# Balajimcr/MuLUT

Measured on AMD Instinct MI355X. Metric: Mpixels/sec SR-x4 2-stage sdy LUT inference (HR output pixels; LR-in = value/16), higher is better.
Workload: dtype u8

## Files before the change

### mulut_amd/_native.py

```python
import ctypes
import os
import shutil
import subprocess

_PKG = os.path.dirname(os.path.abspath(__file__))
_CSRC = os.path.join(_PKG, "csrc")
_LIBDIR = os.path.join(_PKG, "lib")
LIB_PATH = os.path.join(_LIBDIR, "libmulut_hip.so")
SOURCES = ["mulut_kernels.hip", "mulut_k1.hip", "mulut_detail.hip", "mulut_capi.hip", "mulut_ft.hip", "mulut_eval.hip"]
HEADERS = ["mulut_core.h", "mulut_kernels.h", "mulut_dev.h", "mulut_tube2_asm.inc", os.path.join("..", "..", "include", "mulut.h")]
HIPCC_FLAGS = ["--offload-arch=gfx950", "-O3", "-std=c++17", "-fPIC", "-shared", "-Wall", "-Wno-inline-asm", "-Wno-pass-failed"]

EXPORTS = [
    "mulut_version", "mulut_strerror", "mulut_last_hip_error", "mulut_create", "mulut_destroy",
    "mulut_configure", "mulut_set_lut", "mulut_pass", "mulut_stage", "mulut_pipeline",
    "mulut_pipeline_rows", "mulut_halo", "mulut_reserve", "mulut_set_stage_timing", "mulut_last_stage_ms", "mulut_last_kernel_ms",
    "mulut_set_tuning", "mulut_kernel_name", "mulut_ft_stage_forward", "mulut_ft_stage_backward", "mulut_ft_quantize", "mulut_ft_quantize_backward",
    "mulut_ft_stage_forward_mask", "mulut_ft_stage_backward_mask", "mulut_eval_ws_doubles", "mulut_eval_y", "mulut_last_detail_counters", "mulut_debug_read",
]

_libs = {}


def _hipcc():
    return shutil.which("hipcc") or ("/opt/rocm/bin/hipcc" if os.path.exists("/opt/rocm/bin/hipcc") else None)


def source_hash():
    import hashlib
    h = hashlib.sha256()
    for f in sorted(SOURCES + [x for x in HEADERS if not x.endswith("mulut.h")]):
        with open(os.path.join(_CSRC, f), "rb") as fh:
            h.update(fh.read())
    return h.hexdigest()[:16]


def needs_build():
    if not os.path.exists(LIB_PATH):
        return True
    t = os.path.getmtime(LIB_PATH)
    return any(os.path.getmtime(os.path.join(_CSRC, f)) > t for f in SOURCES + HEADERS)


def audit_tube2_isa(asm_path=None):
    import re
    import tempfile
    hipcc = _hipcc()
    if hipcc is None:
        raise RuntimeError("hipcc not found: cannot audit stage_tube2_kernel")
    inc = open(os.path.join(_CSRC, "mulut_tube2_asm.inc")).read()
    row0 = int(re.search(r"#define TUBE2_ROW0 (\d+)", inc).group(1))
    with tempfile.TemporaryDirectory() as td:
        if asm_path is None:
            asm_path = os.path.join(td, "mulut_kernels.s")
            flags = [f for f in HIPCC_FLAGS if f not in ("-fPIC", "-shared")]
            subprocess.check_call([hipcc] + flags + ["--cuda-device-only", "-S", "-o", asm_path, os.path.join(_CSRC, "mulut_kernels.hip")],
                                  stderr=subprocess.DEVNULL)
        lines = open(asm_path).read().splitlines()
    reg = re.compile(r"\bv(\d+)\b|\bv\[(\d+):(\d+)\]")
    kernels, name, in_asm, bad = [], None, False, []
    for line in lines:
        m = re.match(r"^(_ZN5mulut18stage_tube2_kernel\w+):", line)
        if m:
            name, in_asm = m.group(1), False
            kernels.append(name)
            continue
        m = re.match(r"^\s*\.set (_ZN5mulut18stage_tube2_kernel\w+)\.(num_vgpr|num_agpr), (\d+)", line)
        if m:
            if (m.group(2) == "num_agpr" and int(m.group(3)) != 0) or (m.group(2) == "num_vgpr" and int(m.group(3)) > 128):
                bad.append((m.group(1), line.strip()))
            continue
        if name is None:
            continue
        if "s_endpgm" in line:
            name = None
        elif "#ASMSTART" in line:
            in_asm = True
        elif "#ASMEND" in line:
            in_asm = False
        elif not in_asm and not line.lstrip().startswith((";", ".")):
            for a, lo, hi in reg.findall(line.split(";")[0]):
                if (int(a) if a else int(hi)) >= row0:
                    bad.append((name, line.strip()))
    if len(kernels) != 3:
        raise RuntimeError("tube2 audit: expected 3 stage_tube2_kernel instances, found %d" % len(kernels))
    if bad:
        raise RuntimeError("tube2 audit failed (the compiler touched the kernel's private registers, or the register budget changed): %r" % (bad[:5],))
    return len(kernels)


def build(force=False, verbose=False):
    if not force and not needs_build():
        return LIB_PATH
    hipcc = _hipcc()
    if hipcc is None:
        raise RuntimeError("hipcc not found: cannot build libmulut_hip.so (no CPU fallback exists)")
    os.makedirs(_LIBDIR, exist_ok=True)
    tmp = "%s.%d.tmp" % (LIB_PATH, os.getpid())
    cmd = [hipcc] + HIPCC_FLAGS + ["-o", tmp] + SOURCES
    if verbose:
        print(" ".join(cmd))
    try:
        subprocess.check_call(cmd, cwd=_CSRC)
        audit_tube2_isa()
        os.replace(tmp, LIB_PATH)
    finally:
        if os.path.exists(tmp):
            os.remove(tmp)
    return LIB_PATH


def load(path=None):
    path = path or os.environ.get("MULUT_LIB") or LIB_PATH
    if path in _libs:
        return _libs[path]
    if path == LIB_PATH and needs_build():
        if os.environ.get("MULUT_NO_BUILD") == "1":
            if not os.path.exists(LIB_PATH):
                raise RuntimeError("libmulut_hip.so is missing and MULUT_NO_BUILD=1 forbids building it here")
        elif _hipcc() is not None:
            build()
        elif not os.path.exists(LIB_PATH):
            raise RuntimeError("libmulut_hip.so is missing and hipcc is unavailable; "
                               "run `python -c 'import __graft_entry__ as g; g.build()'`")
    L = ctypes.CDLL(path)
    i, p, c_char_p, i64 = ctypes.c_int, ctypes.c_void_p, ctypes.c_char_p, ctypes.c_int64
    L.mulut_version.restype = i
    L.mulut_strerror.argtypes = [i]
    L.mulut_strerror.restype = c_char_p
    L.mulut_last_hip_error.argtypes = [p]
    L.mulut_last_hip_error.restype = c_char_p
    L.mulut_create.argtypes = [i, ctypes.POINTER(p)]
    L.mulut_destroy.argtypes = [p]
    L.mulut_configure.argtypes = [p, i, c_char_p, i, i]
    L.mulut_set_lut.argtypes = [p, i, ctypes.c_char, p, i64, i]
    L.mulut_pass.argtypes = [p, i, ctypes.c_char, i, p, i, i, i, p, p]
    L.mulut_stage.argtypes = [p, i, p, i, p, i, i, i, i, i, p]
    L.mulut_pipeline.argtypes = [p, p, p, i, i, i, i, i, p]
    L.mulut_pipeline_rows.argtypes = [p, p, i, i, p, i, i, i, i, i, i, i, p]
    L.mulut_halo.argtypes = [p]
    L.mulut_reserve.argtypes = [p, i, i, i, i]
    L.mulut_set_stage_timing.argtypes = [p, i]
    L.mulut_last_stage_ms.argtypes = [p, ctypes.POINTER(ctypes.c_float), i]
    L.mulut_last_kernel_ms.argtypes = [p, ctypes.POINTER(ctypes.c_float), i]
    L.mulut_last_detail_counters.argtypes = [p, ctypes.POINTER(ctypes.c_uint32), i, p]
    L.mulut_last_detail_counters.restype = i
    L.mulut_debug_read.argtypes = [p, ctypes.POINTER(ctypes.c_uint64), i, i, p]
    L.mulut_debug_read.restype = i
    L.mulut_set_tuning.argtypes = [p, c_char_p, i]
    L.mulut_kernel_name.argtypes = [p, i]
    L.mulut_ft_stage_forward.argtypes = [i, p, c_char_p, i, i, p, i, i, i, i, p, p]
    L.mulut_ft_stage_backward.argtypes = [i, p, c_char_p, i, i, p, p, i, i, i, i, p, p, p]
    L.mulut_ft_stage_forward_mask.argtypes = [i, p, c_char_p, i, i, p, i, i, i, i, p, p, p]
    L.mulut_ft_stage_backward_mask.argtypes = [i, p, c_char_p, i, i, p, p, p, i, i, i, i, p, p, p]
    L.mulut_kernel_name.restype = c_char_p
    L.mulut_ft_quantize.argtypes = [i, p, p, i, ctypes.c_longlong, p]
    L.mulut_ft_quantize_backward.argtypes = [i, p, p, i, ctypes.c_longlong, p]
    L.mulut_eval_ws_doubles.argtypes = [i, i]
    L.mulut_eval_ws_doubles.restype = ctypes.c_longlong
    L.mulut_eval_y.argtypes = [i, p, p, i, i, i, p, ctypes.c_longlong, ctypes.POINTER(ctypes.c_double),
                               ctypes.POINTER(ctypes.c_double), p]
    L.mulut_eval_y.restype = i
    for name in ("mulut_create", "mulut_destroy", "mulut_configure", "mulut_set_lut", "mulut_pass", "mulut_stage",
                 "mulut_pipeline", "mulut_pipeline_rows", "mulut_halo", "mulut_reserve", "mulut_set_stage_timing",
                 "mulut_last_stage_ms", "mulut_last_kernel_ms", "mulut_set_tuning", "mulut_ft_stage_forward", "mulut_ft_stage_backward",
                 "mulut_ft_quantize", "mulut_ft_quantize_backward", "mulut_ft_stage_forward_mask", "mulut_ft_stage_backward_mask"):
        getattr(L, name).restype = i
    _libs[path] = L
    return L
```

### mulut_amd/csrc/mulut_kernels.hip

```cpp
#include <hip/hip_runtime.h>
#include <string.h>

#include <mutex>
#include <set>
#include <utility>

#include "mulut_dev.h"

namespace mulut {

__global__ void __launch_bounds__(256) pass_kernel(PassArgs a) {
    const long long nsite = (long long)a.C * a.H * a.W;
    const long long s = (long long)blockIdx.x * blockDim.x + threadIdx.x;
    if (s >= nsite) return;
    const int x = (int)(s % a.W);
    const int y = (int)((s / a.W) % a.H);
    const int c = (int)(s / ((long long)a.W * a.H));
    const uint8_t *pl = a.in + (long long)c * a.H * a.W;
    int v[4];
    v[0] = pl[(long long)y * a.W + x];
#pragma unroll
    for (int k = 0; k < 3; ++k) {
        int dy, dx;
        sample_offset(a.r, a.di[k], a.dj[k], dy, dx);
// ... 554 lines not shown
            finish_channel<4, OUT>(a, acc, n, c, y, x, o);
            if constexpr (OUT == kOutPackedRGBU4) {
#pragma unroll
                for (int sy = 0; sy < 4; ++sy) {
                    uint8_t *dst = const_cast<uint8_t *>(view_addr(a.out, n, 0, y * 4 + sy, x * 4)) + c;
#pragma unroll
                    for (int sx = 0; sx < 4; ++sx) dst[3 * sx] = (uint8_t)(o[sy] >> (8 * sx));
                }
            }
        }
    }
}

__global__ void __launch_bounds__(256) stage_up_fix2_kernel(StageArgs a) {
    __shared__ int s_sum[16][16];
    const uint32_t count = *a.fix_count;
    const int grp = (int)(threadIdx.x >> 4), ln = (int)(threadIdx.x & 15);
    const int ylo = imax(a.oy0 - kHalo, 0), yhi = imin(a.oy1 + kHalo, a.H) - 1;
    const int unbias = 128 * kQ * 4 * a.M - a.bias_num;
    for (uint32_t i = blockIdx.x * 16u + (uint32_t)grp; i < count; i += gridDim.x * 16u) {
        const uint32_t ent = a.fix_list[i], id = ent & 0x3FFFFFFFu, only = ent >> 30;
        const int x = (int)(id % (uint32_t)a.W), y = (int)((id / (uint32_t)a.W) % (uint32_t)a.H), n = (int)(id / ((uint32_t)a.W * (uint32_t)a.H));
        if (n >= a.N || y < a.oy0 || y >= a.oy1) continue;
        const int c_lo = only == 3u ? 0 : (int)only, c_hi = only == 3u ? imin(a.C, 3) : imin((int)only + 1, a.C);
        for (int c = c_lo; c < c_hi; ++c) {
            s_sum[grp][ln] = 0;
            __builtin_amdgcn_fence(__ATOMIC_RELEASE, "wavefront");
            auto px = [&](int dy, int dx) {
                const int gy = imin(imax(y + dy, ylo), yhi), gx = imin(imax(x + dx, 0), a.W - 1);
                return (int)*view_addr(a.in, n, c, gy, gx);
            };
            const int va = px(0, 0);
            for (int p = ln; p < 4 * a.M; p += 16) {
                const int m = p >> 2, r = p & 3;
                int dy, dx, v[3];
#pragma unroll
                for (int k = 0; k < 3; ++k) {
                    sample_offset(r, a.di[m][k], a.dj[m][k], dy, dx);
                    v[k] = px(dy, dx);
                }
                int idx[5], w[5];
                simplex4(va, v[0], v[1], v[2], idx, w);
                const uint4 *tab = (const uint4 *)a.lut[m];
                uint32_t row[5][4];
#pragma unroll
                for (int j = 0; j < 5; ++j) {
                    const uint4 t = tab[idx[j]];
                    row[j][0] = t.x; row[j][1] = t.y; row[j][2] = t.z; row[j][3] = t.w;
                }
#pragma unroll
                for (int e = 0; e < 16; ++e) {
                    int sum = 0;
#pragma unroll
                    for (int j = 0; j < 5; ++j) sum += w[j] * (int)((row[j][e >> 2] >> (8 * (e & 3))) & 0xFFu);
                    const int pos = r == 0 ? e : r == 1 ? (e & 3) * 4 + 3 - (e >> 2) : r == 2 ? 15 - e : (3 - (e & 3)) * 4 + (e >> 2);
                    atomicAdd(&s_sum[grp][pos], sum);
                }
            }
            __builtin_amdgcn_fence(__ATOMIC_ACQ_REL, "wavefront");
            const uint32_t b = rhe_clip_u8(s_sum[grp][ln] - unbias, a.div);
            *const_cast<uint8_t *>(view_addr(a.out, n, c, y * 4 + (ln >> 2), x * 4 + (ln & 3))) = (uint8_t)b;
            __builtin_amdgcn_fence(__ATOMIC_ACQ_REL, "wavefront");
        }
    }
}

__global__ void __launch_bounds__(256) stage_up_fix3_kernel(StageArgs a) {
    __shared__ int s_sum[16][16];
    const uint32_t count = *a.fix_count;
    const int grp = (int)(threadIdx.x >> 4), ln = (int)(threadIdx.x & 15);
    const int ylo = imax(a.oy0 - kHalo, 0), yhi = imin(a.oy1 + kHalo, a.H) - 1;
    const int unbias = 128 * kQ * 4 * a.M - a.bias_num;
    const uint32_t stride = gridDim.x * 16u;
    constexpr uint32_t kNone = 0xFFFFFFFFu;
    struct Pix { int x, y, n, va, v[3]; };
    auto decode = [&](uint32_t ent, int &x, int &y, int &n) {
        const uint32_t id = ent & 0x3FFFFFFFu;
        x = (int)(id % (uint32_t)a.W); y = (int)((id / (uint32_t)a.W) % (uint32_t)a.H); n = (int)(id / ((uint32_t)a.W * (uint32_t)a.H));
    };
    auto fetch = [&](uint32_t ent, int c, Pix &p) {
        if (ent == kNone) return;
        decode(ent, p.x, p.y, p.n);
        auto px = [&](int dy, int dx) {
            const int gy = imin(imax(p.y + dy, ylo), yhi), gx = imin(imax(p.x + dx, 0), a.W - 1);
            return (int)*view_addr(a.in, p.n, c, gy, gx);
        };
        p.va = px(0, 0);
        if (ln < 4 * a.M) {
            const int m = ln >> 2, r = ln & 3;
#pragma unroll
            for (int k = 0; k < 3; ++k) {
                int dy, dx;
                sample_offset(r, a.di[m][k], a.dj[m][k], dy, dx);
                p.v[k] = px(dy, dx);
            }
        }
    };
    auto finish = [&](const Pix &p, int c) {
        s_sum[grp][ln] = 0;
        __builtin_amdgcn_fence(__ATOMIC_RELEASE, "wavefront");
        for (int q = ln; q < 4 * a.M; q += 16) {
            const int m = q >> 2, r = q & 3;
            int v[3] = {p.v[0], p.v[1], p.v[2]};
            if (q != ln) {
                auto px = [&](int dy, int dx) {
                    const int gy = imin(imax(p.y + dy, ylo), yhi), gx = imin(imax(p.x + dx, 0), a.W - 1);
                    return (int)*view_addr(a.in, p.n, c, gy, gx);
                };
#pragma unroll
                for (int k = 0; k < 3; ++k) {
                    int dy, dx;
                    sample_offset(r, a.di[m][k], a.dj[m][k], dy, dx);
                    v[k] = px(dy, dx);
                }
            }
            int idx[5], w[5];
            simplex4(p.va, v[0], v[1], v[2], idx, w);
            const uint4 *tab = (const uint4 *)a.lut[m];
            uint32_t row[5][4];
#pragma unroll
            for (int j = 0; j < 5; ++j) {
                const uint4 t = tab[idx[j]];
                row[j][0] = t.x; row[j][1] = t.y; row[j][2] = t.z; row[j][3] = t.w;
            }
#pragma unroll
            for (int e = 0; e < 16; ++e) {
                int sum = 0;
#pragma unroll
                for (int j = 0; j < 5; ++j) sum += w[j] * (int)((row[j][e >> 2] >> (8 * (e & 3))) & 0xFFu);
                const int pos = r == 0 ? e : r == 1 ? (e & 3) * 4 + 3 - (e >> 2) : r == 2 ? 15 - e : (3 - (e & 3)) * 4 + (e >> 2);
                atomicAdd(&s_sum[grp][pos], sum);
            }
        }
        __builtin_amdgcn_fence(__ATOMIC_ACQ_REL, "wavefront");
        const uint32_t b = rhe_clip_u8(s_sum[grp][ln] - unbias, a.div);
        *const_cast<uint8_t *>(view_addr(a.out, p.n, c, p.y * 4 + (ln >> 2), p.x * 4 + (ln & 3))) = (uint8_t)b;
        __builtin_amdgcn_fence(__ATOMIC_ACQ_REL, "wavefront");
    };
    auto first_channel = [&](uint32_t ent) { return (ent >> 30) == 3u ? 0 : (int)(ent >> 30); };

    uint32_t i = blockIdx.x * 16u + (uint32_t)grp;
    uint32_t ent_cur = i < count ? a.fix_list[i] : kNone;
    uint32_t ent_nxt = i + stride < count && i + stride >= i ? a.fix_list[i + stride] : kNone;
    Pix cur, nxt;
    cur.x = cur.y = cur.n = cur.va = 0; cur.v[0] = cur.v[1] = cur.v[2] = 0;
    nxt = cur;
    if (ent_cur != kNone) fetch(ent_cur, first_channel(ent_cur), cur);
    while (ent_cur != kNone) {
        const uint32_t i2 = i + 2u * stride;
        const uint32_t ent_nn = (i2 < count && i2 >= i) ? a.fix_list[i2] : kNone;
        if (ent_nxt != kNone) fetch(ent_nxt, first_channel(ent_nxt), nxt);
        const int c0 = first_channel(ent_cur);
        finish(cur, c0);
        if ((ent_cur >> 30) == 3u)
            for (int c = 1; c < a.C; ++c) {
                Pix p;
                p.v[0] = p.v[1] = p.v[2] = 0;
                fetch(ent_cur, c, p);
                finish(p, c);
            }
        ent_cur = ent_nxt; cur = nxt; ent_nxt = ent_nn; i += stride;
    }
}

hipError_t launch_stage_up_fix(const StageArgs &a, int out_mode, int num_cus, hipStream_t st, int variant) {
    if (a.C > 3 || !a.fix_list || !a.fix_count) return hipErrorInvalidValue;
    const dim3 grid((unsigned)(4 * num_cus)), block(256);
    if (a.M > 4 && variant == 1) variant = 0;
    if (variant == 0) hipLaunchKernelGGL(stage_up_fix2_kernel, dim3((unsigned)(8 * num_cus)), block, 0, st, a);
    else if (variant == 2) hipLaunchKernelGGL(stage_up_fix3_kernel, dim3((unsigned)(8 * num_cus)), block, 0, st, a);
    else if (out_mode == kOutPlanarU4) hipLaunchKernelGGL((stage_up_fix_kernel<kOutPlanarU4>), grid, block, 0, st, a);
    else if (out_mode == kOutPackedRGBU4 && a.C == 3) hipLaunchKernelGGL((stage_up_fix_kernel<kOutPackedRGBU4>), grid, block, 0, st, a);
    else hipLaunchKernelGGL((stage_up_fix_kernel<kOutGeneric>), grid, block, 0, st, a);
    return hipGetLastError();
}

const char *stage_tube_name(int out_mode) {
    return out_mode == kOutPackedRGBU4 ? "stage_tube_kernel<rgb>" : out_mode == kOutPlanarU4 ? "stage_tube_kernel<planar>"
                                                                                              : "stage_tube_kernel<generic>";
}

template <int OUT>
static hipError_t launch_tube_t(const StageArgs &a, const BandArgs &b, int num_cus, hipStream_t st) {
    auto kern = stage_tube_kernel<OUT, KB_TW, KB_TH>;
    {
        const hipError_t e = raise_lds_limit((const void *)kern, 160 * 1024);
        if (e != hipSuccess) return e;
    }
    const long long ntiles = (long long)a.N * a.tiles_x * a.tiles_y;
    if (ntiles <= 0 || ntiles > 0x7fffffffLL) return hipErrorInvalidValue;
    const unsigned grid = (unsigned)(ntiles < num_cus ? ntiles : num_cus);
    hipLaunchKernelGGL(kern, dim3(grid), dim3(KB_TW * KB_TH), (size_t)kTubeLdsBytes, st, a, b);
    return hipGetLastError();
}

hipError_t launch_stage_tube(const StageArgs &a, const BandArgs &b, int out_mode, int num_cus, hipStream_t st) {
    if (a.C > 3 || a.M > 3) return hipErrorInvalidValue;
    if (out_mode == kOutPlanarU4) return launch_tube_t<kOutPlanarU4>(a, b, num_cus, st);
    if (out_mode == kOutPackedRGBU4 && a.C == 3) return launch_tube_t<kOutPackedRGBU4>(a, b, num_cus, st);
    return launch_tube_t<kOutGeneric>(a, b, num_cus, st);
}

#if defined(MULUT_TUBE2_ASM_INC)
#include MULUT_TUBE2_ASM_INC
#else
#include "mulut_tube2_asm.inc"
#endif

struct T2Pair {
    uint32_t base, s0, s1, s2;
    uint32_t w0, w1, w2, w3, w4;
};
__host__ __device__ constexpr int t2_modes(int pats) { return pats & 3; }
__host__ __device__ constexpr int t2_pat(int pats, int m) { return (pats >> (2 + 2 * m)) & 3; }
constexpr int kT2W = 16, kT2H = 4;
constexpr int kT2PW = kT2W + 2 * kTubeHaloX, kT2PH = kT2H + 2 * kHalo, kT2Chan = 2 * kT2PH * kT2PW;
constexpr int kT2WaveTileBytes = 3 * kT2Chan;
constexpr int kT2FixCap = 3 * kT2W * kT2H;
constexpr int kT2FixOff = 3 * kTubeBandBytes + 16 * kT2WaveTileBytes + 2 * 16 * KB_TW * KB_TH;
constexpr int kTube2LdsBytes = kT2FixOff + 16 * kT2FixCap * 4 + 16;
static_assert(kTube2LdsBytes <= 160 * 1024, "LDS budget");
static_assert(KB_TW % kT2W == 0 && KB_TH % kT2H == 0 && (KB_TW / kT2W) * (KB_TH / kT2H) == 16 && KB_TW / kT2W == 4, "16 wave tiles per verdict tile, four across");
__host__ __device__ constexpr int t2_nb(int pat, int r, int k, int sign) {
    return 2 * ((2 + sign * rot_dy(r, kPatDi[pat][k], kPatDj[pat][k])) * kT2PW + 2 + sign * rot_dx(r, kPatDi[pat][k], kPatDj[pat][k]));
}
__host__ __device__ constexpr int t2_imm(int pat) { return pat * kTubeBandBytes - tube_bias(pat); }

__device__ __forceinline__ float t2_f32_of_i16(uint32_t x) {
    float f;
    asm("v_cvt_f32_i32_sdwa %0, sext(%1) dst_sel:DWORD dst_unused:UNUSED_PAD src0_sel:WORD_0" : "=v"(f) : "v"(x));
    return f;
}

template <int PAT>
__device__ __forceinline__ void t2_index(uint32_t k0, uint32_t ha, uint32_t base_a0, uint32_t pb, uint32_t pc, uint32_t pd, T2Pair &o, uint32_t &dirty) {
    constexpr uint32_t SB = kTubeSB * 16, SC = kTubeSC * 16, SD = kTubeSD * 16;
    uint32_t k1 = pb | pk_dup(SB), k2 = pc | pk_dup(SC), k3 = pd | pk_dup(SD);
    const uint32_t hb = pb & 0x000F000Fu, hc = pc & 0x000F000Fu, hd = pd & 0x000F000Fu;
    pk_cmpx_desc(k0, k1);
    pk_cmpx_desc(k2, k3);
    pk_cmpx_desc(k0, k2);
    pk_cmpx_desc(k1, k3);
    pk_cmpx_desc(k1, k2);
    const uint32_t f1 = pk_shr12(k0), f2 = pk_shr12(k1), f3 = pk_shr12(k2), f4 = pk_shr12(k3);
    o.base = pk_mad(pb, pk_dup(SB), pk_mad(pc, pk_dup(SC), pk_mad(pd, pk_dup(SD), base_a0 + pk_dup((uint32_t)tube_bias(PAT)))));
    o.s0 = k0 & 0x0FF00FF0u;
    o.s1 = k1 & 0x0FF00FF0u;
    o.s2 = k2 & 0x0FF00FF0u;
    o.w0 = pk_dup(kQ) - f1;
    o.w1 = f1 - f2;
    o.w2 = f2 - f3;
    o.w3 = f3 - f4;
    o.w4 = f4;
    const uint32_t mx = pk_max(pk_max(hb, hc), pk_max(hd, ha));
    const uint32_t mn = pk_min(pk_min(hb, hc), pk_min(hd, ha));
    dirty |= (mx - mn) & 0xFFFEFFFEu;
}

#define T2_ACC_OPS(lo, hi) [l0] "+v"(lo[0]), [l1] "+v"(lo[1]), [l2] "+v"(lo[2]), [l3] "+v"(lo[3]), [h0] "+v"(hi[0]), [h1] "+v"(hi[1]), [h2] "+v"(hi[2]), [h3] "+v"(hi[3])
#define T2_TMP_OPS [a0] "=&v"(a0), [a1] "=&v"(a1), [a2] "=&v"(a2), [a3] "=&v"(a3)
#define T2_W_OPS(c) [w0] "v"(c.w0), [w1] "v"(c.w1), [w2] "v"(c.w2), [w3] "v"(c.w3), [w4] "v"(c.w4)
#define T2_ADDR_OPS(n) [base] "v"(n.base), [s0] "v"(n.s0), [s1] "v"(n.s1), [s2] "v"(n.s2)
#define T2_IMM_OPS(PAT) [ilo] "i"(t2_imm(PAT)), [ihi] "i"(t2_imm(PAT) + kTubePlaneBytes), [ilo4] "i"(t2_imm(PAT) + kTubeAll * 16), [ihi4] "i"(t2_imm(PAT) + kTubeAll * 16 + kTubePlaneBytes)
#define T2_NB_OPS(PAT, R, OFF) [n0] "i"(t2_nb(PAT, R, 0, 1) + (OFF)), [n1] "i"(t2_nb(PAT, R, 0, -1) + (OFF)), [n2] "i"(t2_nb(PAT, R, 1, 1) + (OFF)), \
    [n3] "i"(t2_nb(PAT, R, 1, -1) + (OFF)), [n4] "i"(t2_nb(PAT, R, 2, 1) + (OFF)), [n5] "i"(t2_nb(PAT, R, 2, -1) + (OFF)), [nan] "i"(2 * (2 * kT2PW + 2) + (OFF))

#define T2_NBOUT_OPS [pb] "=&v"(pb), [pc] "=&v"(pc), [pd] "=&v"(pd), [t0] "=&v"(t0), [t1] "=&v"(t1), [t2] "=&v"(t2)
template <int PAT>
__device__ __forceinline__ void t2_block_a(uint32_t (&lo)[4], uint32_t (&hi)[4], const T2Pair &cur) {
    uint32_t a0, a1, a2, a3;
    asm volatile(TUBE2_ASM_A : T2_ACC_OPS(lo, hi), T2_TMP_OPS : T2_W_OPS(cur), T2_ADDR_OPS(cur), T2_IMM_OPS(PAT) : TUBE2_CLOBBERS);
}
template <int NPAT, int NN, int TPAT, int TR, int TOFF, bool LAST>
__device__ __forceinline__ void t2_block_b(uint32_t (&lo)[4], uint32_t (&hi)[4], const T2Pair &cur, const T2Pair &nxt, uint32_t win,
                                           uint32_t &pb, uint32_t &pc, uint32_t &pd, uint32_t &ca) {
    uint32_t a0, a1, a2, a3, t0, t1, t2;
    if constexpr (LAST)
        asm volatile(TUBE2_ASM_B_LAST : T2_ACC_OPS(lo, hi) : T2_W_OPS(cur) : TUBE2_CLOBBERS);
    else if constexpr (NN == 0)
        asm volatile(TUBE2_ASM_B_N0 : T2_ACC_OPS(lo, hi), T2_TMP_OPS : T2_W_OPS(cur), T2_ADDR_OPS(nxt), T2_IMM_OPS(NPAT) : TUBE2_CLOBBERS);
    else if constexpr (NN == 6)
        asm volatile(TUBE2_ASM_B_N6 : T2_ACC_OPS(lo, hi), T2_TMP_OPS, T2_NBOUT_OPS : T2_W_OPS(cur), T2_ADDR_OPS(nxt), T2_IMM_OPS(NPAT), [win] "v"(win), T2_NB_OPS(TPAT, TR, TOFF) : TUBE2_CLOBBERS);
    else
        asm volatile(TUBE2_ASM_B_N7 : T2_ACC_OPS(lo, hi), T2_TMP_OPS, T2_NBOUT_OPS, [ca] "=&v"(ca) : T2_W_OPS(cur), T2_ADDR_OPS(nxt), T2_IMM_OPS(NPAT), [win] "v"(win), T2_NB_OPS(TPAT, TR, TOFF) : TUBE2_CLOBBERS);
}

template <int OUT, int PATS>
__global__ void __launch_bounds__(KB_TW *KB_TH) __attribute__((amdgpu_waves_per_eu(TUBE2_WAVES_PER_EU, TUBE2_WAVES_PER_EU))) stage_tube2_kernel(StageArgs a, BandArgs b) {
    constexpr int TW = KB_TW, TH = KB_TH, PW = kT2PW, PH = kT2PH, NT = TW * TH;
    constexpr int M = t2_modes(PATS), NP = 2 * M;
    constexpr int DW = PW / 4, PER4 = (3 * PH * DW + 63) / 64;
    extern __shared__ __attribute__((aligned(16))) uint8_t smem[];
    uint32_t *s_next = (uint32_t *)(smem + kTube2LdsBytes - 16);
    if (lds_addr_of(smem) != 0u) __builtin_trap();

    const int ntiles = a.N * a.tiles_x * a.tiles_y;
    const int G = gridDim.x;
    const bool by_xcd = (G & 7) == 0;
    const int per = (ntiles + 7) >> 3;
    const int first = by_xcd ? (int)(blockIdx.x & 7) * per + (int)(blockIdx.x >> 3) : (int)blockIdx.x;
    const int last = by_xcd ? imin(((int)(blockIdx.x & 7) + 1) * per, ntiles) : ntiles;
    const int step = by_xcd ? (G >> 3) : G;
    if (first >= last) return;
    const int ylo = imax(a.oy0 - kHalo, 0), yhi = imin(a.oy1 + kHalo, a.H) - 1;
    const bool dw_ok = __builtin_amdgcn_readfirstlane((int)(a.in.sX == 1 && ((a.W | a.in.sY | a.in.sC) & 3) == 0 && (a.in.sN & 3) == 0 && (((uintptr_t)a.in.p) & 3) == 0)) != 0;
    const int wave = __builtin_amdgcn_readfirstlane((int)(threadIdx.x >> 6));
    uint8_t *img = smem + 3 * kTubeBandBytes + wave * kT2WaveTileBytes;

    auto grab = [&]() {
        for (;;) {
            uint32_t j = 0;
            if ((threadIdx.x & 63) == 0) j = atomicAdd(s_next, 1u);
            j = (uint32_t)__builtin_amdgcn_readfirstlane((int)j);
            const long long tile = (long long)first + (long long)(j >> 4) * step;
            if (tile >= last) return -1;
            if (a.verdict_take >= 0 && (int)a.verdict[tile] != a.verdict_take) continue;
            int n, ty0, tx0;
            decode_tile(a, (int)tile, n, ty0, tx0, TW, TH);
            if (tx0 + kT2W * (int)(j & 3u) >= a.W || ty0 + kT2H * (int)((j >> 2) & 3u) >= a.oy1) continue;
            return (int)j;
        }
    };
    auto origin = [&](int j, int &n, int &y0, int &x0) {
        decode_tile(a, first + (j >> 4) * step, n, y0, x0, TW, TH);
        x0 += kT2W * (j & 3);
        y0 += kT2H * ((j >> 2) & 3);
    };
    auto fetch = [&](int j, uint32_t (&v)[PER4]) {
        if (!dw_ok || j < 0) return;
        int n, y0, x0;
        origin(j, n, y0, x0);
        int lane = (int)(threadIdx.x & 63);
        asm volatile("" : "+v"(lane));
#pragma unroll
        for (int k = 0; k < PER4; ++k) {
            const int i = lane + 64 * k;
            const int q = i % DW, py = (i / DW) % PH, c = imin(i / (DW * PH), a.C - 1);
            const int gy = imin(imax(y0 + py - kHalo, ylo), yhi);
            const int gx = imin(imax(x0 - kTubeHaloX + 4 * q, 0), a.W - 4);
            v[k] = *(const uint32_t *)view_addr(a.in, n, c, gy, gx);
        }
    };
    auto stash = [&](int j, const uint32_t (&v)[PER4]) {
        if (j < 0) return;
        int n, y0, x0;
        origin(j, n, y0, x0);
        int lane = (int)(threadIdx.x & 63);
        asm volatile("" : "+v"(lane));
        if (dw_ok) {
            const bool edge = __builtin_amdgcn_readfirstlane((int)(x0 - kTubeHaloX < 0 || x0 - kTubeHaloX + 4 * (DW - 1) > a.W - 4)) != 0;
#pragma unroll
            for (int k = 0; k < PER4; ++k) {
                const int i = lane + 64 * k;
                if (i < a.C * PH * DW) {
                    uint32_t lo, hi;
                    if (!edge) {
                        lo = __builtin_amdgcn_perm(0u, v[k], 0x0C010C00u); hi = __builtin_amdgcn_perm(0u, v[k], 0x0C030C02u);
                    } else {
                        const int gx = x0 - kTubeHaloX + 4 * (i % DW);
                        const uint32_t sel_lo = gx < 0 ? 0x0C000C00u : gx > a.W - 4 ? 0x0C030C03u : 0x0C010C00u;
                        const uint32_t sel_hi = gx < 0 ? 0x0C000C00u : gx > a.W - 4 ? 0x0C030C03u : 0x0C030C02u;
                        lo = __builtin_amdgcn_perm(0u, v[k], sel_lo); hi = __builtin_amdgcn_perm(0u, v[k], sel_hi);
                    }
                    uint2 c2;
                    c2.x = pk_mad(lo, pk_dup(0x1000u), pk_shr4(lo));
                    c2.y = pk_mad(hi, pk_dup(0x1000u), pk_shr4(hi));
                    *(uint2 *)(img + 8 * i) = c2;
                }
            }
        } else {
            for (int i = lane; i < a.C * PH * PW; i += 64) {
                const int px = i % PW, py = (i / PW) % PH, c = i / (PW * PH);
                const int gy = imin(imax(y0 + py - kHalo, ylo), yhi);
                const int gx = imin(imax(x0 + px - kTubeHaloX, 0), a.W - 1);
                ((uint16_t *)img)[i] = (uint16_t)pixel_code1(*view_addr(a.in, n, c, gy, gx));
            }
        }
    };

#if defined(MULUT_VARIANT_t2prof)
    const unsigned long long t_first = __builtin_amdgcn_s_memtime(), r_first = __builtin_amdgcn_s_memrealtime();
    uint32_t t_prev = (uint32_t)t_first, t_ph0 = 0, t_ph1 = 0, t_ph2 = 0, t_ph3 = 0, t_ph4 = 0, t_ph5 = 0;
#define T2_STAMP(PH) do { const uint32_t t_now = (uint32_t)__builtin_amdgcn_s_memtime(); t_ph##PH += t_now - t_prev; t_prev = t_now; } while (0)
#elif defined(MULUT_T2_MARKERS)
#define T2_STAMP(PH) asm volatile("; MULUT_T2_PHASE_END " #PH)
#else
#define T2_STAMP(PH) do { } while (0)
#endif
    static_for<0, M>([&](auto MI) {
        constexpr int pat = t2_pat(PATS, MI);
        const uint4 *src = (const uint4 *)b.band[MI];
        uint4 *dst = (uint4 *)(smem + pat * kTubeBandBytes);
        const uint32_t k = b.scale[MI];
        if (k == 0x00010001u) {
            for (int i = threadIdx.x; i < kTubeBandBytes / 16; i += NT) dst[i] = src[i];
        } else {
            for (int i = threadIdx.x; i < kTubeBandBytes / 16; i += NT) {
                const uint4 v = src[i];
                dst[i] = make_uint4(pk_mad(v.x, k, 0u), pk_mad(v.y, k, 0u), pk_mad(v.z, k, 0u), pk_mad(v.w, k, 0u));
            }
        }
    });
    if (threadIdx.x == 0) *s_next = 0u;
    __syncthreads();
    T2_STAMP(5);

    uint32_t *fix_buf = (uint32_t *)(smem + kT2FixOff) + wave * kT2FixCap;
    uint32_t fix_have = 0u;
    auto fix_flush = [&]() {
        if (fix_have == 0u) return;
        const unsigned long long act = __ballot(true);
        const uint32_t rank = (uint32_t)__popcll(act & ((1ull << (threadIdx.x & 63)) - 1ull)), nact = (uint32_t)__popcll(act);
        uint32_t at = 0u;
        if (rank == 0u) at = atomicAdd(a.fix_count, fix_have);
        at = (uint32_t)__builtin_amdgcn_readfirstlane((int)at);
        __builtin_amdgcn_fence(__ATOMIC_ACQ_REL, "wavefront");
        for (uint32_t i = rank; i < fix_have; i += nact) a.fix_list[at + i] = fix_buf[i];
        __builtin_amdgcn_fence(__ATOMIC_ACQ_REL, "wavefront");
        fix_have = 0u;
    };
    uint32_t pix[PER4];
    int item = grab();
    fetch(item, pix);
    stash(item, pix);
    while (item >= 0) {
        const int nxt_item = grab();
        fetch(nxt_item, pix);
        auto site = [&](int &n_, int &y_, int &x_, int &lx_, int &ly_) {
            int y0, x0;
            origin(item, n_, y0, x0);
            int l = (int)(threadIdx.x & 63);
            asm volatile("" : "+v"(l));
            lx_ = l % kT2W; ly_ = l / kT2W;
            y_ = y0 + ly_; x_ = x0 + lx_;
        };
        int n, y, x, lx, ly;
        site(n, y, x, lx, ly);
        T2_STAMP(0);
        if (y < a.oy1 && x < a.W) {
            uint32_t win = (uint32_t)(3 * kTubeBandBytes + wave * kT2WaveTileBytes + 2 * (ly * PW + lx + kTubeHaloX - kHalo));
            auto park = [&]() {
                int t = (int)threadIdx.x;
                asm volatile("" : "+v"(t));
                return (uint4 *)(smem + 3 * kTubeBandBytes + 16 * kT2WaveTileBytes) + t;
            };
            uint32_t dmask = 0u, dirty = 0u, dirty_n = 0u;
            uint32_t o[4] = {0u, 0u, 0u, 0u};
            uint32_t pb, pc, pd, ca;
            uint32_t k0, ha, ba0;
            auto anchor = [&](uint32_t c2) {
                k0 = (c2 & 0xF000F000u) | pk_dup((uint32_t)kTubeSA * 16);
                ha = c2 & 0x000F000Fu;
                ba0 = pk_mad(c2, pk_dup((uint32_t)kTubeSA * 16), 0u);
            };
            T2Pair cur, nxt;
            {
                constexpr int p0 = t2_pat(PATS, 0);
                uint32_t t0, t1, t2;
                asm volatile(TUBE2_ASM_LOAD_NB_ANCHOR : T2_NBOUT_OPS, [ca] "=&v"(ca) : [win] "v"(win), T2_NB_OPS(p0, 0, 0) : TUBE2_CLOBBERS);
                anchor(ca);
                t2_index<p0>(k0, ha, ba0, pb, pc, pd, cur, dirty);
                asm volatile(TUBE2_ASM_LOAD_NB : T2_NBOUT_OPS : [win] "v"(win), T2_NB_OPS(p0, 1, 0) : TUBE2_CLOBBERS);
                uint32_t a0, a1, a2, a3;
                asm volatile(TUBE2_ASM_FIRST_ROWS : T2_TMP_OPS : T2_ADDR_OPS(cur), T2_IMM_OPS(p0) : TUBE2_CLOBBERS);
                t2_index<p0>(k0, ha, ba0, pb, pc, pd, nxt, dirty);
            }
            RotAcc<4> acc;
            const bool wide = a.M > 4;
            auto acc_start = [&]() {
                acc.clear();
                if (OUT != kOutGeneric && !wide) {
                    const uint32_t nb = pk_dup((uint32_t)(65536 - 128 * kQ * 4 * a.M));
#pragma unroll
                    for (int k = 0; k < 4; ++k) acc.lo02[k] = acc.hi02[k] = nb;
                }
            };
            acc_start();
            T2_STAMP(1);
#pragma clang loop unroll(disable)
            for (int c = 0; c < a.C; ++c, win += kT2Chan) {
                const bool more = c + 1 < a.C;
                asm volatile("; MULUT_T2_STREAM_BEGIN (tools/ubench/gen_stream_ubench.py cuts the ISA here)");
                static_for<0, NP>([&](auto PI) {
                    constexpr int p = PI;
                    if constexpr (p == (NP >= 6 ? 4 : NP - 1)) asm volatile("; MULUT_T2_STREAM_END");
                    constexpr int pat = t2_pat(PATS, p >> 1), R = p & 1;
                    constexpr bool t_here = p + 2 < NP;
                    constexpr int tp = t_here ? p + 2 : p + 2 - NP, tpat = t2_pat(PATS, tp >> 1), tr = tp & 1, toff = t_here ? 0 : kT2Chan;
                    constexpr bool n_here = p + 1 < NP;
                    constexpr int npat = t2_pat(PATS, n_here ? (p + 1) >> 1 : 0);
                    T2Pair nn;
                    auto &lo = R == 0 ? acc.lo02 : acc.lo13;
                    auto &hi = R == 0 ? acc.hi02 : acc.hi13;
                    t2_block_a<pat>(lo, hi, cur);
                    if (t_here || more) {
                        t2_block_b<npat, (tp == 0 ? 7 : 6), tpat, tr, toff, false>(lo, hi, cur, nxt, win, pb, pc, pd, ca);
                        if constexpr (tp == 0) anchor(ca);
                        if constexpr (t_here) t2_index<tpat>(k0, ha, ba0, pb, pc, pd, nn, dirty);
                        else t2_index<tpat>(k0, ha, ba0, pb, pc, pd, nn, dirty_n);
                    } else {
                        if constexpr (n_here) t2_block_b<npat, 0, 0, 0, 0, false>(lo, hi, cur, nxt, win, pb, pc, pd, ca);
                        else t2_block_b<npat, 0, 0, 0, 0, true>(lo, hi, cur, nxt, win, pb, pc, pd, ca);
                        nn = nxt;
                    }
                    cur = nxt;
                    nxt = nn;
                });
                if (wide) {
                    tube_finish_rows_wide(a, acc, o);
                    if constexpr (OUT == kOutPackedRGBU4) {
                        if (c < 2) park()[c * NT] = make_uint4(o[0], o[1], o[2], o[3]);
                    } else {
                        int n2, y2, x2, lx2, ly2;
                        site(n2, y2, x2, lx2, ly2);
#pragma unroll
                        for (int sy = 0; sy < 4; ++sy) {
                            if constexpr (OUT == kOutPlanarU4) {
                                *(uint32_t *)const_cast<uint8_t *>(view_addr(a.out, n2, c, y2 * 4 + sy, x2 * 4)) = o[sy];
                            } else {
#pragma unroll
                                for (int sx = 0; sx < 4; ++sx) *const_cast<uint8_t *>(view_addr(a.out, n2, c, y2 * 4 + sy, x2 * 4 + sx)) = (uint8_t)(o[sy] >> (8 * sx));
                            }
                        }
                    }
                } else if constexpr (OUT != kOutGeneric) {
                    static_for<0, 4>([&](auto SY) {
                        constexpr int sy = SY;
                        const uint32_t s0 = tube_field<4 * sy + 0>(acc.lo02, acc.hi02) + tube_field<12 + sy>(acc.lo13, acc.hi13);
                        const uint32_t s1 = tube_field<4 * sy + 1>(acc.lo02, acc.hi02) + tube_field<8 + sy>(acc.lo13, acc.hi13);
                        const uint32_t s2 = tube_field<4 * sy + 2>(acc.lo02, acc.hi02) + tube_field<4 + sy>(acc.lo13, acc.hi13);
                        const uint32_t s3 = tube_field<4 * sy + 3>(acc.lo02, acc.hi02) + tube_field<0 + sy>(acc.lo13, acc.hi13);
                        uint32_t r = __builtin_amdgcn_cvt_pk_u8_f32(t2_f32_of_i16(s0) * a.inv_d, 0u, 0u);
                        r = __builtin_amdgcn_cvt_pk_u8_f32(t2_f32_of_i16(s1) * a.inv_d, 1u, r);
                        r = __builtin_amdgcn_cvt_pk_u8_f32(t2_f32_of_i16(s2) * a.inv_d, 2u, r);
                        r = __builtin_amdgcn_cvt_pk_u8_f32(t2_f32_of_i16(s3) * a.inv_d, 3u, r);
                        o[sy] = r;
                    });
                    if constexpr (OUT == kOutPackedRGBU4) {
                        if (c < 2) park()[c * NT] = make_uint4(o[0], o[1], o[2], o[3]);
                    } else {
                        int n2, y2, x2, lx2, ly2;
                        site(n2, y2, x2, lx2, ly2);
#pragma unroll
                        for (int sy = 0; sy < 4; ++sy) *(uint32_t *)const_cast<uint8_t *>(view_addr(a.out, n2, c, y2 * 4 + sy, x2 * 4)) = o[sy];
                    }
                } else {
                    int n2, y2, x2, lx2, ly2;
                    site(n2, y2, x2, lx2, ly2);
                    finish_channel<4, OUT>(a, acc, n2, c, y2, x2, o);
                }
                acc_start();
                dmask |= (dirty != 0u ? 1u : 0u) << c;
                dirty = dirty_n;
                dirty_n = 0u;
            }
            T2_STAMP(2);
            site(n, y, x, lx, ly);
            if constexpr (OUT == kOutPackedRGBU4) {
                const uint4 r = park()[0], g = park()[NT];
                const uint32_t oR[4] = {r.x, r.y, r.z, r.w}, oG[4] = {g.x, g.y, g.z, g.w};
                store_rgb<4>(a, n, y, x, oR, oG, o);
            }
#if defined(MULUT_VARIANT_nofixlist)
            if (dmask == 0xFFFFFFFFu) a.fix_list[0] = 0u;
#else
            if (__ballot(dmask != 0u) != 0ull) {
                const uint32_t pixel_id = (uint32_t)((n * a.H + y) * a.W + x);
                const unsigned long long m0 = __ballot((dmask & 1u) != 0u), m1 = __ballot((dmask & 2u) != 0u), m2 = __ballot((dmask & 4u) != 0u);
                const uint32_t n0 = (uint32_t)__popcll(m0), n1 = (uint32_t)__popcll(m1), n2 = (uint32_t)__popcll(m2);
                if (fix_have + n0 + n1 + n2 > (uint32_t)kT2FixCap) fix_flush();
                const unsigned long long below = (1ull << (threadIdx.x & 63)) - 1ull;
                if (dmask & 1u) fix_buf[fix_have + (uint32_t)__popcll(m0 & below)] = pixel_id;
                if (dmask & 2u) fix_buf[fix_have + n0 + (uint32_t)__popcll(m1 & below)] = pixel_id | (1u << 30);
                if (dmask & 4u) fix_buf[fix_have + n0 + n1 + (uint32_t)__popcll(m2 & below)] = pixel_id | (2u << 30);
                fix_have += n0 + n1 + n2;
            }
#endif
        }
        T2_STAMP(3);
        stash(nxt_item, pix);
        T2_STAMP(4);
        item = nxt_item;
    }
    fix_flush();
#if defined(MULUT_VARIANT_t2prof)
    if (a.dbg && (threadIdx.x & 63) == 0) {
        atomicAdd(a.dbg + 0, (unsigned long long)t_ph0); atomicAdd(a.dbg + 1, (unsigned long long)t_ph1); atomicAdd(a.dbg + 2, (unsigned long long)t_ph2);
        atomicAdd(a.dbg + 3, (unsigned long long)t_ph3); atomicAdd(a.dbg + 4, (unsigned long long)t_ph4); atomicAdd(a.dbg + 5, (unsigned long long)t_ph5);
        atomicAdd(a.dbg + 6, __builtin_amdgcn_s_memtime() - t_first);
        atomicAdd(a.dbg + 7, __builtin_amdgcn_s_memrealtime() - r_first);
        atomicAdd(a.dbg + 8, 1ull);
    }
#endif
#undef T2_STAMP
}

constexpr int kT2PatsSDY = 3 | (0 << 2) | (1 << 4) | (2 << 6);

static bool tube2_counts(const StageArgs &a, int (&cnt)[3]) {
    cnt[0] = cnt[1] = cnt[2] = 0;
    for (int m = 0; m < a.M; ++m) {
        int di[3], dj[3], p = -1;
        for (int q = 0; q < 3 && p < 0; ++q) {
            pattern_offsets("sdy"[q], di, dj);
            if (memcmp(di, a.di[m], sizeof(di)) == 0 && memcmp(dj, a.dj[m], sizeof(dj)) == 0) p = q;
        }
        if (p < 0) return false;
        ++cnt[p];
    }
    return true;
}
bool stage_tube2_supported(const StageArgs &a) {
    int cnt[3];
    return a.C <= 3 && a.M <= kMaxTube2Modes && tube2_counts(a, cnt) && cnt[0] && cnt[1] && cnt[2] && (a.M > 4 || a.use_f32) &&
           a.bias_num == 0;
}

template <int OUT>
static hipError_t launch_tube2_t(const StageArgs &a, const BandArgs &b, int num_cus, hipStream_t st) {
    auto kern = stage_tube2_kernel<OUT, kT2PatsSDY>;
    {
        const hipError_t e = raise_lds_limit((const void *)kern, 160 * 1024);
        if (e != hipSuccess) return e;
    }
    const long long ntiles = (long long)a.N * a.tiles_x * a.tiles_y;
    if (ntiles <= 0 || ntiles > 0x7fffffffLL) return hipErrorInvalidValue;
    const unsigned grid = (unsigned)(ntiles < num_cus ? ntiles : num_cus);
    hipLaunchKernelGGL(kern, dim3(grid), dim3(KB_TW * KB_TH), (size_t)kTube2LdsBytes, st, a, b);
    return hipGetLastError();
}

hipError_t launch_stage_tube2(const StageArgs &a, const BandArgs &bm, int out_mode, int num_cus, hipStream_t st) {
    int cnt[3];
    if (!stage_tube2_supported(a) || !tube2_counts(a, cnt)) return hipErrorInvalidValue;
    BandArgs b;
    memset(&b, 0, sizeof(b));
    for (int m = 0; m < a.M; ++m) {
        const int p = a.dj[m][0] == 2 ? 1 : a.di[m][0] == 1 ? 2 : 0;
        b.band[p] = bm.band[m];
        b.scale[p] = (uint32_t)cnt[p] * 0x00010001u;
    }
    if (out_mode == kOutPlanarU4) return launch_tube2_t<kOutPlanarU4>(a, b, num_cus, st);
    if (out_mode == kOutPackedRGBU4 && a.C == 3) return launch_tube2_t<kOutPackedRGBU4>(a, b, num_cus, st);
    return launch_tube2_t<kOutGeneric>(a, b, num_cus, st);
}

}
```

Measured before the change: 144,100.

## Reload tube2 kernel args from kernarg segment to cut SGPR/VGPR pressure

Replaces values held across the tube2 loop (dw_ok, ylo/yhi, decoded tile bases) with on-demand scalar loads from the kernarg segment pointer. Fetch and stash now use one lane per (row, dword) with a per-channel inner loop, and output addresses use 32-bit offsets with inlined RGB interleaved stores. The fix-list flush assumes a full wave and the ballot is moved outside the in-bounds branch so all lanes take part. The aim is lower register pressure and cheaper address math, at the cost of more scalar loads and a new restriction that the batch strides fit in 31 bits.

```diff
diff --git a/mulut_amd/_native.py b/mulut_amd/_native.py
--- a/mulut_amd/_native.py
+++ b/mulut_amd/_native.py
@@ -72,7 +72,7 @@
             continue
         if name is None:
             continue
-        if "s_endpgm" in line:
+        if line.startswith(".Lfunc_end"):
             name = None
         elif "#ASMSTART" in line:
             in_asm = True
diff --git a/mulut_amd/csrc/mulut_kernels.hip b/mulut_amd/csrc/mulut_kernels.hip
--- a/mulut_amd/csrc/mulut_kernels.hip
+++ b/mulut_amd/csrc/mulut_kernels.hip
@@ -880,11 +880,30 @@
     const int last = by_xcd ? imin(((int)(blockIdx.x & 7) + 1) * per, ntiles) : ntiles;
     const int step = by_xcd ? (G >> 3) : G;
     if (first >= last) return;
-    const int ylo = imax(a.oy0 - kHalo, 0), yhi = imin(a.oy1 + kHalo, a.H) - 1;
-    const bool dw_ok = __builtin_amdgcn_readfirstlane((int)(a.in.sX == 1 && ((a.W | a.in.sY | a.in.sC) & 3) == 0 && (a.in.sN & 3) == 0 && (((uintptr_t)a.in.p) & 3) == 0)) != 0;
+    typedef const __attribute__((address_space(4))) StageArgs KArgs;
+    auto kargs = [&]() {
+        uint64_t p = (uint64_t)(uintptr_t)__builtin_amdgcn_kernarg_segment_ptr();
+        asm volatile("" : "+s"(p));
+        const uint32_t lo = (uint32_t)__builtin_amdgcn_readfirstlane((int)(uint32_t)p), hi = (uint32_t)__builtin_amdgcn_readfirstlane((int)(uint32_t)(p >> 32));
+        return (KArgs *)(uintptr_t)(((uint64_t)hi << 32) | lo);
+    };
+    auto dw_ok = [&]() {
+        KArgs *k = kargs();
+        return k->in.sX == 1 && ((k->W | k->in.sY | k->in.sC) & 3) == 0 && (k->in.sN & 3) == 0 && (((uintptr_t)k->in.p) & 3) == 0;
+    };
     const int wave = __builtin_amdgcn_readfirstlane((int)(threadIdx.x >> 6));
     uint8_t *img = smem + 3 * kTubeBandBytes + wave * kT2WaveTileBytes;
 
+    auto origin = [&](int j, int &n, int &y0, int &x0) {
+        KArgs *k = kargs();
+        int b = first + (j >> 4) * step;
+        const int tx = b % k->tiles_x;
+        b /= k->tiles_x;
+        const int ty = b % k->tiles_y;
+        n = b / k->tiles_y;
+        y0 = k->oy0 + ty * TH + kT2H * ((j >> 2) & 3);
+        x0 = tx * TW + kT2W * (j & 3);
+    };
     auto grab = [&]() {
         for (;;) {
             uint32_t j = 0;
@@ -892,61 +911,67 @@
             j = (uint32_t)__builtin_amdgcn_readfirstlane((int)j);
             const long long tile = (long long)first + (long long)(j >> 4) * step;
             if (tile >= last) return -1;
-            if (a.verdict_take >= 0 && (int)a.verdict[tile] != a.verdict_take) continue;
-            int n, ty0, tx0;
-            decode_tile(a, (int)tile, n, ty0, tx0, TW, TH);
-            if (tx0 + kT2W * (int)(j & 3u) >= a.W || ty0 + kT2H * (int)((j >> 2) & 3u) >= a.oy1) continue;
+            KArgs *k = kargs();
+            if (k->verdict_take >= 0 && (int)k->verdict[tile] != k->verdict_take) continue;
+            int n, y0, x0;
+            origin((int)j, n, y0, x0);
+            if (x0 >= k->W || y0 >= k->oy1) continue;
             return (int)j;
         }
     };
-    auto origin = [&](int j, int &n, int &y0, int &x0) {
-        decode_tile(a, first + (j >> 4) * step, n, y0, x0, TW, TH);
-        x0 += kT2W * (j & 3);
-        y0 += kT2H * ((j >> 2) & 3);
-    };
+    static_assert(PH * 8 == 64 && DW <= 8 && PER4 == 3, "one lane per (image row, dword) of a channel; one dword per channel and lane");
     auto fetch = [&](int j, uint32_t (&v)[PER4]) {
-        if (!dw_ok || j < 0) return;
+        if (j < 0 || !dw_ok()) return;
         int n, y0, x0;
         origin(j, n, y0, x0);
-        int lane = (int)(threadIdx.x & 63);
+        KArgs *k = kargs();
+        const int ylo = imax(k->oy0 - kHalo, 0), yhi = imin(k->oy1 + kHalo, k->H) - 1;
+        uint32_t lane = threadIdx.x & 63u;
         asm volatile("" : "+v"(lane));
-#pragma unroll
-        for (int k = 0; k < PER4; ++k) {
-            const int i = lane + 64 * k;
-            const int q = i % DW, py = (i / DW) % PH, c = imin(i / (DW * PH), a.C - 1);
-            const int gy = imin(imax(y0 + py - kHalo, ylo), yhi);
-            const int gx = imin(imax(x0 - kTubeHaloX + 4 * q, 0), a.W - 4);
-            v[k] = *(const uint32_t *)view_addr(a.in, n, c, gy, gx);
+        const uint32_t q = lane & 7u, py = lane >> 3;
+        if (q < (uint32_t)DW) {
+            const int gy = imin(imax(y0 + (int)py - kHalo, ylo), yhi);
+            const int gx = imin(imax(x0 - kTubeHaloX + 4 * (int)q, 0), k->W - 4);
+            const uint32_t off = (uint32_t)(gy - k->in.row0) * (uint32_t)k->in.sY + (uint32_t)gx;
+            const uint8_t *plane = k->in.p + (long long)n * k->in.sN;
+#pragma unroll
+            for (int c = 0; c < PER4; ++c) v[c] = *(const uint32_t *)(plane + (long long)imin(c, k->C - 1) * k->in.sC + off);
         }
     };
     auto stash = [&](int j, const uint32_t (&v)[PER4]) {
         if (j < 0) return;
         int n, y0, x0;
         origin(j, n, y0, x0);
-        int lane = (int)(threadIdx.x & 63);
-        asm volatile("" : "+v"(lane));
-        if (dw_ok) {
-            const bool edge = __builtin_amdgcn_readfirstlane((int)(x0 - kTubeHaloX < 0 || x0 - kTubeHaloX + 4 * (DW - 1) > a.W - 4)) != 0;
-#pragma unroll
-            for (int k = 0; k < PER4; ++k) {
-                const int i = lane + 64 * k;
-                if (i < a.C * PH * DW) {
-                    uint32_t lo, hi;
-                    if (!edge) {
-                        lo = __builtin_amdgcn_perm(0u, v[k], 0x0C010C00u); hi = __builtin_amdgcn_perm(0u, v[k], 0x0C030C02u);
-                    } else {
-                        const int gx = x0 - kTubeHaloX + 4 * (i % DW);
-                        const uint32_t sel_lo = gx < 0 ? 0x0C000C00u : gx > a.W - 4 ? 0x0C030C03u : 0x0C010C00u;
-                        const uint32_t sel_hi = gx < 0 ? 0x0C000C00u : gx > a.W - 4 ? 0x0C030C03u : 0x0C030C02u;
-                        lo = __builtin_amdgcn_perm(0u, v[k], sel_lo); hi = __builtin_amdgcn_perm(0u, v[k], sel_hi);
+        KArgs *k = kargs();
+        if (dw_ok()) {
+            uint32_t lane = threadIdx.x & 63u;
+            asm volatile("" : "+v"(lane));
+            const uint32_t q = lane & 7u, py = lane >> 3;
+            if (q < (uint32_t)DW) {
+                const int W = k->W;
+                const bool edge = x0 - kTubeHaloX < 0 || x0 - kTubeHaloX + 4 * (DW - 1) > W - 4;
+                uint32_t sel_lo = 0x0C010C00u, sel_hi = 0x0C030C02u;
+                if (edge) {
+                    const int gx = x0 - kTubeHaloX + 4 * (int)q;
+                    sel_lo = gx < 0 ? 0x0C000C00u : gx > W - 4 ? 0x0C030C03u : 0x0C010C00u;
+                    sel_hi = gx < 0 ? 0x0C000C00u : gx > W - 4 ? 0x0C030C03u : 0x0C030C02u;
+                }
+                uint2 *dst = (uint2 *)img + (py * DW + q);
+#pragma unroll
+                for (int c = 0; c < PER4; ++c) {
+                    if (c < k->C) {
+                        const uint32_t lo = __builtin_amdgcn_perm(0u, v[c], sel_lo), hi = __builtin_amdgcn_perm(0u, v[c], sel_hi);
+                        uint2 c2;
+                        c2.x = pk_mad(lo, pk_dup(0x1000u), pk_shr4(lo));
+                        c2.y = pk_mad(hi, pk_dup(0x1000u), pk_shr4(hi));
+                        dst[c * PH * DW] = c2;
                     }
-                    uint2 c2;
-                    c2.x = pk_mad(lo, pk_dup(0x1000u), pk_shr4(lo));
-                    c2.y = pk_mad(hi, pk_dup(0x1000u), pk_shr4(hi));
-                    *(uint2 *)(img + 8 * i) = c2;
                 }
             }
         } else {
+            int lane = (int)(threadIdx.x & 63);
+            asm volatile("" : "+v"(lane));
+            const int ylo = imax(a.oy0 - kHalo, 0), yhi = imin(a.oy1 + kHalo, a.H) - 1;
             for (int i = lane; i < a.C * PH * PW; i += 64) {
                 const int px = i % PW, py = (i / PW) % PH, c = i / (PW * PH);
                 const int gy = imin(imax(y0 + py - kHalo, ylo), yhi);
@@ -987,8 +1012,7 @@
     uint32_t fix_have = 0u;
     auto fix_flush = [&]() {
         if (fix_have == 0u) return;
-        const unsigned long long act = __ballot(true);
-        const uint32_t rank = (uint32_t)__popcll(act & ((1ull << (threadIdx.x & 63)) - 1ull)), nact = (uint32_t)__popcll(act);
+        const uint32_t rank = threadIdx.x & 63u, nact = 64u;
         uint32_t at = 0u;
         if (rank == 0u) at = atomicAdd(a.fix_count, fix_have);
         at = (uint32_t)__builtin_amdgcn_readfirstlane((int)at);
@@ -996,6 +1020,10 @@
         for (uint32_t i = rank; i < fix_have; i += nact) a.fix_list[at + i] = fix_buf[i];
         __builtin_amdgcn_fence(__ATOMIC_ACQ_REL, "wavefront");
         fix_have = 0u;
+    };
+    auto out_off = [&](int y_, int x_) {
+        KArgs *k = kargs();
+        return (uint32_t)(4 * y_ - k->out.row0) * (uint32_t)k->out.sY + (uint32_t)(4 * x_) * (uint32_t)k->out.sX;
     };
     uint32_t pix[PER4];
     int item = grab();
@@ -1015,6 +1043,7 @@
         int n, y, x, lx, ly;
         site(n, y, x, lx, ly);
         T2_STAMP(0);
+        uint32_t dmask = 0u;
         if (y < a.oy1 && x < a.W) {
             uint32_t win = (uint32_t)(3 * kTubeBandBytes + wave * kT2WaveTileBytes + 2 * (ly * PW + lx + kTubeHaloX - kHalo));
             auto park = [&]() {
@@ -1022,7 +1051,7 @@
                 asm volatile("" : "+v"(t));
                 return (uint4 *)(smem + 3 * kTubeBandBytes + 16 * kT2WaveTileBytes) + t;
             };
-            uint32_t dmask = 0u, dirty = 0u, dirty_n = 0u;
+            uint32_t dirty = 0u, dirty_n = 0u;
             uint32_t o[4] = {0u, 0u, 0u, 0u};
             uint32_t pb, pc, pd, ca;
             uint32_t k0, ha, ba0;
@@ -1120,7 +1149,7 @@
                         int n2, y2, x2, lx2, ly2;
                         site(n2, y2, x2, lx2, ly2);
 #pragma unroll
-                        for (int sy = 0; sy < 4; ++sy) *(uint32_t *)const_cast<uint8_t *>(view_addr(a.out, n2, c, y2 * 4 + sy, x2 * 4)) = o[sy];
+                        for (int sy = 0; sy < 4; ++sy) *(uint32_t *)(a.out.p + (long long)n2 * a.out.sN + (long long)c * a.out.sC + (out_off(y2, x2) + (uint32_t)sy * (uint32_t)a.out.sY)) = o[sy];
                     }
                 } else {
                     int n2, y2, x2, lx2, ly2;
@@ -1137,24 +1166,36 @@
             if constexpr (OUT == kOutPackedRGBU4) {
                 const uint4 r = park()[0], g = park()[NT];
                 const uint32_t oR[4] = {r.x, r.y, r.z, r.w}, oG[4] = {g.x, g.y, g.z, g.w};
-                store_rgb<4>(a, n, y, x, oR, oG, o);
-            }
+                KArgs *k = kargs();
+                uint8_t *plane = k->out.p + (long long)n * k->out.sN;
+                const uint32_t off = out_off(y, x), sY = (uint32_t)k->out.sY;
+#pragma unroll
+                for (int sy = 0; sy < 4; ++sy) {
+                    uint32_t w0, w1, w2;
+                    interleave_rgb4(oR[sy], oG[sy], o[sy], w0, w1, w2);
+                    uint32_t *dst = (uint32_t *)(plane + (off + (uint32_t)sy * sY));
+                    dst[0] = w0;
+                    dst[1] = w1;
+                    dst[2] = w2;
+                }
+            }
+        }
 #if defined(MULUT_VARIANT_nofixlist)
-            if (dmask == 0xFFFFFFFFu) a.fix_list[0] = 0u;
+        if (dmask == 0xFFFFFFFFu) a.fix_list[0] = 0u;
 #else
-            if (__ballot(dmask != 0u) != 0ull) {
-                const uint32_t pixel_id = (uint32_t)((n * a.H + y) * a.W + x);
-                const unsigned long long m0 = __ballot((dmask & 1u) != 0u), m1 = __ballot((dmask & 2u) != 0u), m2 = __ballot((dmask & 4u) != 0u);
-                const uint32_t n0 = (uint32_t)__popcll(m0), n1 = (uint32_t)__popcll(m1), n2 = (uint32_t)__popcll(m2);
-                if (fix_have + n0 + n1 + n2 > (uint32_t)kT2FixCap) fix_flush();
-                const unsigned long long below = (1ull << (threadIdx.x & 63)) - 1ull;
-                if (dmask & 1u) fix_buf[fix_have + (uint32_t)__popcll(m0 & below)] = pixel_id;
-                if (dmask & 2u) fix_buf[fix_have + n0 + (uint32_t)__popcll(m1 & below)] = pixel_id | (1u << 30);
-                if (dmask & 4u) fix_buf[fix_have + n0 + n1 + (uint32_t)__popcll(m2 & below)] = pixel_id | (2u << 30);
-                fix_have += n0 + n1 + n2;
-            }
+        if (__ballot(dmask != 0u) != 0ull) {
+            KArgs *k = kargs();
+            const uint32_t pixel_id = ((uint32_t)n * (uint32_t)k->H + (uint32_t)y) * (uint32_t)k->W + (uint32_t)x;
+            const unsigned long long m0 = __ballot((dmask & 1u) != 0u), m1 = __ballot((dmask & 2u) != 0u), m2 = __ballot((dmask & 4u) != 0u);
+            const uint32_t n0 = (uint32_t)__popcll(m0), n1 = (uint32_t)__popcll(m1), n2 = (uint32_t)__popcll(m2);
+            if (fix_have + n0 + n1 + n2 > (uint32_t)kT2FixCap) fix_flush();
+            const unsigned long long below = (1ull << (threadIdx.x & 63)) - 1ull;
+            if (dmask & 1u) fix_buf[fix_have + (uint32_t)__popcll(m0 & below)] = pixel_id;
+            if (dmask & 2u) fix_buf[fix_have + n0 + (uint32_t)__popcll(m1 & below)] = pixel_id | (1u << 30);
+            if (dmask & 4u) fix_buf[fix_have + n0 + n1 + (uint32_t)__popcll(m2 & below)] = pixel_id | (2u << 30);
+            fix_have += n0 + n1 + n2;
+        }
 #endif
-        }
         T2_STAMP(3);
         stash(nxt_item, pix);
         T2_STAMP(4);
@@ -1191,7 +1232,7 @@
 bool stage_tube2_supported(const StageArgs &a) {
     int cnt[3];
     return a.C <= 3 && a.M <= kMaxTube2Modes && tube2_counts(a, cnt) && cnt[0] && cnt[1] && cnt[2] && (a.M > 4 || a.use_f32) &&
-           a.bias_num == 0;
+           a.bias_num == 0 && a.in.sN > 0 && a.in.sN < (1LL << 31) && a.out.sN > 0 && a.out.sN < (1LL << 31);
 }
 
 template <int OUT>
```

After: 144,800, median of 6. No clear change (+0.5%).
